# se-hwan/landing-controller

Hardware: AMD Instinct MI355X
Metric: landing NLPs solved/sec (SRBM, N=40, batch) (higher is better)
Workload: dtype f64

## Files before the change

landing-controller_amd/csrc/layout.hpp:

```cpp
#pragma once

namespace landing {

struct Layout {
  int N;
  int nx, ng, np, nnz_jac, nnz_hess;
  int o_dt, o_q_min, o_q_max, o_qd_min, o_qd_max, o_q_init, o_qd_init, o_q_term_min, o_q_term_max,
      o_qd_term_min, o_qd_term_max, o_QN, o_mu, o_l_leg_max, o_f_max, o_mass, o_Ib, o_Ib_inv;
  int o_Uref, o_QX, o_Qc, o_Qf;
  double kin_box[3], kin_z_off, comp_eps, slip_eps;
  int run_cost;
  double QX[12], Qc[3], Qf[3], f_ref[3], p_hip[12];

  __host__ __device__ int x_X(int k) const { return 12 * k; }
  __host__ __device__ int x_U(int k) const { return 12 * (N + 1) + 24 * k; }
  __host__ __device__ int g_stage(int k) const { return 36 + 104 * k; }
  __host__ __device__ int rows(int k) const { return k == N - 1 ? 80 : 104; }
  __host__ __device__ int jx(int k) const { return 157 * k; }
  __host__ __device__ int ju(int k) const { return 157 * N + 36 + (k == 0 ? 0 : 204 + 228 * (k - 1)); }
  __host__ __device__ int ju_len(int k) const { return k == 0 ? (N == 1 ? 156 : 204) : (k == N - 1 ? 180 : 228); }
  __host__ __device__ int hx(int k) const { return 29 * k; }
  __host__ __device__ int hu(int k) const { return 29 * N + 12 + (k == 0 ? 0 : 148 + 160 * (k - 1)); }
};

inline Layout make_layout(int N) {
  Layout L;
  L.N = N;
  L.nx = 36 * N + 12; L.ng = 104 * N + 12; L.np = 13 * N + 94;
  L.nnz_jac = 36 + 385 * (N - 1) + 313; L.nnz_hess = 177 * N + 12 * (N - 1) + 12;
  L.o_dt = 12 * (N + 1);
  const int b = L.o_dt + N;
  L.o_q_min = b; L.o_q_max = b + 6; L.o_qd_min = b + 12; L.o_qd_max = b + 18; L.o_q_init = b + 24; L.o_qd_init = b + 30;
  L.o_q_term_min = b + 36; L.o_q_term_max = b + 42; L.o_qd_term_min = b + 48; L.o_qd_term_max = b + 54;
  L.o_QN = b + 60; L.o_mu = b + 72; L.o_l_leg_max = b + 73; L.o_f_max = b + 74; L.o_mass = b + 75; L.o_Ib = b + 76; L.o_Ib_inv = b + 79;
  L.kin_box[0] = 0.15; L.kin_box[1] = 0.15; L.kin_box[2] = 0.30; L.kin_z_off = 0.05; L.comp_eps = 1e-3; L.slip_eps = 1e-2;
  L.run_cost = 0;
  L.o_Uref = L.o_QX = L.o_Qc = L.o_Qf = -1;
  { const double ph[12] = {0.19, -0.1, -0.2, 0.19, 0.1, -0.2, -0.19, -0.1, -0.2, -0.19, 0.1, -0.2};
    for (int i = 0; i < 12; ++i) { L.QX[i] = 0.0; L.p_hip[i] = ph[i]; }
    for (int i = 0; i < 3; ++i) { L.Qc[i] = 0.0; L.Qf[i] = 0.0; L.f_ref[i] = 0.0; } }
  return L;
}

inline void layout_ccc_params(Layout& L) {
  const int N = L.N;
  L.run_cost = 2;
  L.o_Uref = 12 * (N + 1);
  L.o_dt = L.o_Uref + 24 * N;
  const int b = L.o_dt + N;
  L.o_q_min = b; L.o_q_max = b + 6; L.o_qd_min = b + 12; L.o_qd_max = b + 18; L.o_q_init = b + 24; L.o_qd_init = b + 30;
  L.o_q_term_min = b + 36; L.o_q_term_max = b + 42; L.o_qd_term_min = b + 48; L.o_qd_term_max = b + 54;
  L.o_QX = b + 60; L.o_QN = b + 72; L.o_Qc = b + 84; L.o_Qf = b + 87;
  L.o_mu = b + 90; L.o_l_leg_max = b + 91; L.o_f_max = b + 92; L.o_mass = b + 93; L.o_Ib = b + 94; L.o_Ib_inv = b + 97;
  L.np = b + 100;
}

}
```

landing-controller_amd/csrc/solver_kernels.hip:

```cpp
#include <hip/hip_runtime.h>
#include <math.h>
#include <type_traits>

#include "../../include/landing_nlp.h"
#include "ipm_core.hpp"


namespace landing {

constexpr int NZ_JX = 0, NZ_JU = 157, NZ_JUN = 385, NZ_HX = 613, NZ_HU = 642, NZ_HUN = 802, NZ_TOT = 962;
constexpr int GS = 49;
constexpr int PS = 25;
constexpr int YS = 37;
constexpr int RIC_K = 0, RIC_KAP = 576, RIC_MT = 600, RIC_MV = 888, RIC_PX = 900, RIC_PV = 1188, RIC_STRIDE = 1200;
constexpr int RIC_FWD0 = 288, RIC_FWDN = 612;
constexpr int FILT_CAP = 64;
constexpr int SOLVER_NMAX = 96;
constexpr int SOLVER_THREADS = 256;
constexpr int RCG = 36;
constexpr int RUNC = 48;

constexpr int CX_SR = NZ_TOT + 48, CX_ONE = CX_SR + 208, CX_MONE = CX_ONE + 1, CX_ZERO = CX_ONE + 2, CX_LEN = CX_ONE + 3;
constexpr int ATAB_TB = 6, ATAB_LTMAX = 6;
constexpr int ASM_NSLOT = 512;
// ... 107 lines not shown
#pragma unroll
  for (int i = 0; i < MEMBER_MEM_PTRS; ++i) {
    const unsigned long long a = (unsigned long long)q[i];
    const unsigned lo = (unsigned)__builtin_amdgcn_readfirstlane((int)(unsigned)a), hi = (unsigned)__builtin_amdgcn_readfirstlane((int)(unsigned)(a >> 32));
    q[i] = (double*)((unsigned long long)lo | ((unsigned long long)hi << 32));
  }
#endif
  return M;
}
static_assert(36 * FWD_DXL_NMAX + 12 <= 24 * PS + 2 * XCH + 2 * 12 * YS && offsetof(Lds, A1) == offsetof(Lds, P) + sizeof(double) * 24 * PS && offsetof(Lds, Ah) == offsetof(Lds, A1) + sizeof(double) * 2 * XCH,
              "dx (x layout, N <= FWD_DXL_NMAX) fits the adjacent arrays [P | A1 | A^] (forward_pass / row_products)");
static_assert(offsetof(Lds, atab_mid) <= 65528, "the assembly tables address G, A^, gamma, cx, the partial sums and the dump slots with 16-bit byte offsets");
__host__ __device__ inline unsigned long long aterm_pack(int pa, int pb, int pc, int d, bool keep, bool ah) {
  const unsigned lo = (unsigned)pa | ((unsigned)pb << 16);
  const unsigned hi = (unsigned)pc | (((unsigned)d | (keep ? 1u : 0u) | (ah ? 2u : 0u)) << 16);
  return (unsigned long long)lo | ((unsigned long long)hi << 32);
}
__host__ __device__ inline unsigned long long acomb_pack(int n, int s0, int d, bool ah) {
  return (unsigned long long)((unsigned)n | ((unsigned)s0 << 16)) | ((unsigned long long)((unsigned)d | (ah ? 2u : 0u)) << 32);
}

template <int KT, class FA, class FB>
__device__ __forceinline__ f64x4 mfma_tile(f64x4 c, FA fa, FB fb) {
  const int l = threadIdx.x & 63, ij = l & 15, kq = l >> 4;
#pragma unroll
  for (int kt = 0; kt < KT; ++kt) c = __builtin_amdgcn_mfma_f64_16x16x4f64(fa(ij, kt * 4 + kq), fb(kt * 4 + kq, ij), c, 0, 0, 0);
  return c;
}

__device__ __forceinline__ double fast_rcp(double d) {
  double i = __builtin_amdgcn_rcp(d);
  i = fma(i, fma(-d, i, 1.0), i);
  return fma(i, fma(-d, i, 1.0), i);
}

__device__ __forceinline__ double lane_bcast(double v, int src) {
  const int hi = __builtin_amdgcn_readlane(__double2hiint(v), src);
  const int lo = __builtin_amdgcn_readlane(__double2loint(v), src);
  return __hiloint2double(hi, lo);
}

template <int NU>
__device__ __noinline__ void gauss_jordan_wave(const double* G, const double* gam, double* Kl, double* kl, int* flag) {
  const int lane = threadIdx.x;
  double col[NU];
  const bool isUU = lane < NU, isUS = lane >= NU && lane < NU + 24, isG = lane == NU + 24;
  {
    const double* src = isG ? gam + 24 : G + 24 * GS + (isUU ? 24 + lane : (isUS ? lane - NU : 0));
    const int stride = isG ? 1 : GS;
#pragma unroll
    for (int i = 0; i < NU; ++i) col[i] = src[i * stride];
  }
  bool ok = true;
#pragma unroll 1
  for (int j = 0; j < NU; ++j) {
    const double d = lane_bcast(col[0], j);
    if (!(d > 0.0) || !(d < 1e300)) ok = false;
    double inv = __builtin_amdgcn_rcp(d);
    inv = fma(inv, fma(-d, inv, 1.0), inv);
    inv = fma(inv, fma(-d, inv, 1.0), inv);
    const double pj = col[0] * inv;
    double m[NU];
#pragma unroll
    for (int i = 1; i < NU; ++i) m[i] = lane_bcast(col[i], j);
    __builtin_amdgcn_sched_barrier(0);
#pragma unroll
    for (int i = 1; i < NU; ++i) col[i - 1] = fma(-m[i], pj, col[i]);
    col[NU - 1] = pj;
  }
  if (isUS) {
#pragma unroll
    for (int i = 0; i < NU; ++i) Kl[i * 24 + (lane - NU)] = col[i];
  }
  if (isG) {
#pragma unroll
    for (int i = 0; i < NU; ++i) kl[i] = col[i];
  }
  if (lane == 0) *flag = ok ? 1 : 0;
}

constexpr int ASM_SEG_LEN[7] = {NZ_JU - NZ_JX, NZ_JUN - NZ_JU, NZ_HX - NZ_JUN, NZ_HU - NZ_HX, NZ_HUN - NZ_HU, NZ_TOT - NZ_HUN, RUNC};
constexpr int ASM_SEG_POS[7] = {NZ_JX, NZ_JU, NZ_JUN, NZ_HX, NZ_HU, NZ_HUN, NZ_TOT};
static_assert(NZ_JUN - NZ_JU <= SOLVER_THREADS && 2 * 104 <= SOLVER_THREADS, "one load per thread and segment");
struct AsmRegs { double jh[7], sr, g, rc; };
__device__ __forceinline__ void asm_issue(int k, AsmRegs& R) {
  const Lds& S = SH;
  const MemberMem& M = S.M;
  const int tid = threadIdx.x, ng = S.L.ng;
  landing_gptr JH = (landing_gptr)M.J;
  landing_gptr SR = (landing_gptr)M.sig;
  const int* sb = S.segb + k * 8;
  const int g0 = S.L.g_stage(k);
#pragma unroll
  for (int sgm = 0; sgm < 7; ++sgm) R.jh[sgm] = JH[sb[sgm] + (tid < ASM_SEG_LEN[sgm] ? tid : 0)];
  R.sr = SR[tid < 104 ? g0 + tid : (tid < 208 ? ng + g0 + tid - 104 : 0)];
  R.g = ((landing_gptr)M.g)[g0 + (tid < 12 ? tid : 0)];
  R.rc = 0.0;
  if (S.rc_on) R.rc = ((landing_gptr)M.cond)[(size_t)k * RCG + (tid < RCG ? tid : 0)];
}
__device__ __forceinline__ void asm_copy(const AsmRegs& R) {
  Lds& S = SH;
  const int tid = threadIdx.x;
#pragma unroll
  for (int sgm = 0; sgm < 7; ++sgm) if (tid < ASM_SEG_LEN[sgm]) S.jhl[ASM_SEG_POS[sgm] + tid] = R.jh[sgm];
  if (tid < 208) S.jhl[CX_SR + tid] = R.sr;
}
__device__ __forceinline__ void asm_terms(int k, int nb, const AsmRegs& R) {
  Lds& S = SH;
  const int tid = threadIdx.x, LT = S.c_ml, tp = S.segb[k * 8 + 7];
  char* const lds0 = reinterpret_cast<char*>(&S);
  const unsigned ahoff = nb ? (unsigned)(12 * YS * sizeof(double)) : 0u;
  const bool mid = (tp == S.c_mid);
  const unsigned long long* gt = S.ctab + (size_t)tp * LT * SOLVER_THREADS;
  double acc = 0.0;
  for (int j0 = 0; j0 < LT; j0 += ATAB_TB) {
    unsigned long long t[ATAB_TB];
    if (mid) {
#pragma unroll
      for (int u = 0; u < ATAB_TB; ++u) t[u] = S.atab_mid[(j0 + u) * SOLVER_THREADS + tid];
    } else {
#pragma unroll
      for (int u = 0; u < ATAB_TB; ++u) t[u] = gt[(j0 + u) * SOLVER_THREADS + tid];
    }
    double a[ATAB_TB], b[ATAB_TB], c[ATAB_TB];
#pragma unroll
    for (int u = 0; u < ATAB_TB; ++u) {
      const unsigned lo = (unsigned)t[u], hi = (unsigned)(t[u] >> 32);
      a[u] = *reinterpret_cast<const double*>(lds0 + (lo & 0xffffu)); b[u] = *reinterpret_cast<const double*>(lds0 + (lo >> 16)); c[u] = *reinterpret_cast<const double*>(lds0 + (hi & 0xffffu));
    }
#pragma unroll
    for (int u = 0; u < ATAB_TB; ++u) {
      const unsigned dd = (unsigned)(t[u] >> 48);
      acc += a[u] * b[u] * c[u];
      *reinterpret_cast<double*>(lds0 + ((dd & 0xfff8u) + ((dd & 2u) ? ahoff : 0u))) = acc;
      acc = (dd & 1u) ? acc : 0.0;
    }
  }
  if (tid < 12) { const int i = tid; S.Ah[nb * (12 * YS) + (i < 6 ? i : (i < 9 ? i + 3 : i - 3)) * YS + (YS - 1)] = -R.g; }
  if (tid < RCG) S.rcl[tid] = R.rc;
}
__device__ __forceinline__ void asm_combine(int k, int nb) {
  Lds& S = SH;
  const int tid = threadIdx.x, tp = S.segb[k * 8 + 7];
  const unsigned long long code = tp == S.c_mid ? S.acomb_mid[tid] : S.ccomb[tp * SOLVER_THREADS + tid];
  const unsigned lo = (unsigned)code, dd = (unsigned)(code >> 32);
  const int n = (int)(lo & 7u);
  if (n > 0) {
    char* const lds0 = reinterpret_cast<char*>(&S);
    const double* sl = reinterpret_cast<const double*>(lds0 + (lo >> 16));
    double tot = 0.0;
    for (int i = 0; i < n; ++i) tot += sl[i];
    *reinterpret_cast<double*>(lds0 + ((dd & 0xfff8u) + ((dd & 2u) ? (nb ? (unsigned)(12 * YS * sizeof(double)) : 0u) : 0u))) = tot;
  }
}

#if defined(__HIP_DEVICE_COMPILE__)
typedef double __attribute__((address_space(1)))* landing_gptr_w;
#else
typedef double* landing_gptr_w;
#endif
__device__ __forceinline__ landing_gptr_w uniform_record(double* rec) {
#if defined(__HIP_DEVICE_COMPILE__)
  const unsigned long long a = (unsigned long long)rec;
  const unsigned lo = (unsigned)__builtin_amdgcn_readfirstlane((int)(unsigned)a), hi = (unsigned)__builtin_amdgcn_readfirstlane((int)(unsigned)(a >> 32));
  return (landing_gptr_w)((unsigned long long)lo | ((unsigned long long)hi << 32));
#else
  return rec;
#endif
}

template <int STEP>
__device__ __forceinline__ bool pivot_block_step(f64x4 (&T)[3], int ct, int lj, int lk, int c) {
  constexpr int OFF = 4 * STEP;
  static_assert((OFF >> 4) == ((OFF + 3) >> 4), "a pivot block lies inside one row tile");
  Lds& S = SH;
  constexpr int RTB = OFF >> 4, R0 = (OFF & 15) >> 2;
  constexpr int WSZ = 64 * 4;
  static_assert(WSZ + 48 * 4 <= XCH, "exchange buffer");
  double* W = S.A1 + (STEP & 1) * XCH;
  double* C = W + WSZ;
#pragma unroll
  for (int q = 0; q < 1; ++q) W[c * 4 + 4 * q + lk] = T[RTB][R0 + q];
  if (ct == RTB && lj >= (OFF & 15) && lj < (OFF & 15) + 4) {
#pragma unroll
    for (int rt = 0; rt < 3; ++rt)
#pragma unroll
      for (int r = 0; r < 4; ++r) C[(16 * rt + lk + 4 * r) * 4 + (lj - (OFF & 15))] = T[rt][r];
  }
  __syncthreads();
  double a[4][4];
#pragma unroll
  for (int i = 0; i < 4; ++i)
#pragma unroll
    for (int j = 0; j <= i; ++j) a[i][j] = C[(OFF + i) * 4 + j];
  double w[4];
#pragma unroll
  for (int i = 0; i < 4; ++i) w[i] = W[c * 4 + i];
  double am[3];
#pragma unroll
  for (int rt = 0; rt < 3; ++rt) { const int row = 16 * rt + lj; const double cv = C[row * 4 + lk]; am[rt] = (row >= OFF && row < OFF + 4) ? 0.0 : cv; }
  auto recip = [](double d) { double i = __builtin_amdgcn_rcp(d); i = fma(i, fma(-d, i, 1.0), i); return fma(i, fma(-d, i, 1.0), i); };
  const double a00 = a[0][0], a10 = a[1][0], a11 = a[1][1], a20 = a[2][0], a21 = a[2][1], a22 = a[2][2], a30 = a[3][0], a31 = a[3][1], a32 = a[3][2], a33 = a[3][3];
  const double detA = fma(a00, a11, -a10 * a10), iA = recip(detA);
  const double e00 = fma(a20, a11, -a21 * a10) * iA, e01 = fma(a21, a00, -a20 * a10) * iA, e10 = fma(a30, a11, -a31 * a10) * iA, e11 = fma(a31, a00, -a30 * a10) * iA;
  const double s00 = fma(-e01, a21, fma(-e00, a20, a22)), s10 = fma(-e11, a21, fma(-e10, a20, a32)), s11 = fma(-e11, a31, fma(-e10, a30, a33));
  const double detS = fma(s00, s11, -s10 * s10), iS = recip(detS);
  unsigned hm = 0u;
  { const double piv[4] = {a00, detA, s00, detS};
#pragma unroll
    for (int j = 0; j < 4; ++j) { const unsigned h = (unsigned)__double2hiint(piv[j]) - 0x00100000u; hm = h > hm ? h : hm; } }
  const bool ok = hm < (0x7e37e43cu - 0x00100000u);
  auto solve = [&](const double (&wv)[4]) {
    const double t2 = fma(-e01, wv[1], fma(-e00, wv[0], wv[2])), t3 = fma(-e11, wv[1], fma(-e10, wv[0], wv[3]));
    const double r2 = fma(s11, t2, -s10 * t3) * iS, r3 = fma(s00, t3, -s10 * t2) * iS;
    const double q0 = fma(a11, wv[0], -a10 * wv[1]) * iA, q1 = fma(a00, wv[1], -a10 * wv[0]) * iA;
    const double r0 = fma(-e10, r3, fma(-e00, r2, q0)), r1 = fma(-e11, r3, fma(-e01, r2, q1));
    return lk == 0 ? r0 : (lk == 1 ? r1 : (lk == 2 ? r2 : r3));
  };
  const double R = solve(w);
  if (16 * ct + 16 > OFF) {
#pragma unroll
    for (int rt = 0; rt < 3; ++rt) T[rt] = __builtin_amdgcn_mfma_f64_16x16x4f64(am[rt], -R, T[rt], 0, 0, 0);
    T[RTB][R0] = R;
  }
  return ok;
}

constexpr int G_GAMMA = GS - 1, P_PV = PS - 1, AH_B = YS - 1;
static_assert(G_GAMMA == 48 && P_PV == 24 && AH_B == 36, "spare columns of G / P / A^ hold gamma / p / b");
template <int NU>
__device__ __noinline__ bool block_eliminate(double* __restrict__ rec_, double delta, int k) {
  Lds& S = SH;
  constexpr int NR = NU + 24;
  const int tid = threadIdx.x, ct = tid >> 6, l = tid & 63, lj = l & 15, lk = l >> 4;
  const int c = 16 * ct + lj;
  const bool isg = (c == NR), live = (c <= NR);
  const int cb = k & 1;
  f64x4 T[3];
  const double* const lds0 = reinterpret_cast<const double*>(&S);
  constexpr int oG = (int)(offsetof(Lds, G) / sizeof(double)), oP = (int)(offsetof(Lds, P) / sizeof(double));
  const int oAh = (int)(offsetof(Lds, Ah) / sizeof(double)) + cb * (12 * YS);
  const int cl = c < NR ? c : NR;
  const int cp = NU == 24 ? cl : (cl < NU ? cl : cl + (24 - NU));
  const bool ym = live && (c < 12 || c >= NU);
  int ycol = c < NU ? c + 24 : c - NU;
  ycol = ym ? (isg ? AH_B : ycol) : 0;
  const bool pm = live && c >= 12 && (c < NU || isg);
  const int pcol = pm ? (isg ? P_PV : c) : 0;
  {
    const int gb = oG + cp + lk * GS, cd = cp - lk, cm = c - lk;
#pragma unroll
    for (int rt = 0; rt < 3; ++rt)
#pragma unroll
      for (int r = 0; r < 4; ++r) {
        const int rb = 16 * rt + 4 * r;
        if (rb < NR) {
          const int rp = NU == 24 ? rb : (rb < NU ? rb : rb + (24 - NU));
          const int m = rp < cd ? rp : cd;
          const double v = lds0[gb + rp + (GS - 1) * m] + (cm == rb ? delta : 0.0);
          T[rt][r] = live ? v : 0.0;
        } else T[rt][r] = 0.0;
      }
    if (S.rc_on) {
#pragma unroll
      for (int rt = 0; rt < 3; ++rt)
#pragma unroll
        for (int r = 0; r < 4; ++r) {
          const int rb = 16 * rt + 4 * r;
          if (rb < NR) {
            const int ab = rb < NU ? 24 + rb : rb - NU;
            static_assert(RCG % 4 == 0 && NU % 4 == 0, "a group of four rows lies on one side of every border");
            const double g = ab < RCG ? S.rcl[ab + lk] : 0.0;
            T[rt][r] += isg ? g : 0.0;
          }
        }
    }
  }
  {
    double be[3];
    {
      const int yb = oAh + lk * YS + ycol;
#pragma unroll
      for (int kt = 0; kt < 3; ++kt) { const double v = lds0[yb + 4 * kt * YS]; be[kt] = ym ? v : 0.0; }
    }
    double pa1[3], add1[3];
#pragma unroll
    for (int kt = 0; kt < 3; ++kt) pa1[kt] = lds0[oP + lj * PS + 4 * kt + lk];
    const int pb = oP + lk * PS + pcol;
#pragma unroll
    for (int r = 0; r < 3; ++r) { const double v = lds0[pb + 4 * r * PS]; add1[r] = pm ? v : 0.0; }
    double av[3][3];
#pragma unroll
    for (int rt = 0; rt < 3; ++rt) {
      const int rho = 16 * rt + lj;
      const int a = rho < NU ? 24 + rho : (rho < NR ? rho - NU : 36);
      const bool am = a < 36;
      const int ab = oAh + lk * YS + (am ? a : 0);
#pragma unroll
      for (int kt = 0; kt < 3; ++kt) { const double v = lds0[ab + 4 * kt * YS]; av[rt][kt] = am ? v : 0.0; }
    }
    double pa2[3], add2[3];
    if (NU == 24) {
      const int p2 = oP + (12 + (lj < 12 ? lj : 11)) * PS + lk;
#pragma unroll
      for (int kt = 0; kt < 3; ++kt) pa2[kt] = lds0[p2 + 4 * kt];
#pragma unroll
      for (int r = 0; r < 3; ++r) { const double v = lds0[pb + (12 + 4 * r) * PS]; add2[r] = pm ? v : 0.0; }
    }
    f64x4 Y1 = {0.0, 0.0, 0.0, 0.0};
#pragma unroll
    for (int kt = 0; kt < 3; ++kt) Y1 = __builtin_amdgcn_mfma_f64_16x16x4f64(pa1[kt], be[kt], Y1, 0, 0, 0);
#pragma unroll
    for (int r = 0; r < 3; ++r) Y1[r] += add1[r];
#pragma unroll
    for (int rt = 0; rt < 3; ++rt)
#pragma unroll
      for (int kt = 0; kt < 3; ++kt) T[rt] = __builtin_amdgcn_mfma_f64_16x16x4f64(av[rt][kt], Y1[kt], T[rt], 0, 0, 0);
    if (NU == 24) {
      f64x4 Y2 = {0.0, 0.0, 0.0, 0.0};
#pragma unroll
      for (int kt = 0; kt < 3; ++kt) Y2 = __builtin_amdgcn_mfma_f64_16x16x4f64(pa2[kt], be[kt], Y2, 0, 0, 0);
#pragma unroll
      for (int r = 0; r < 3; ++r) Y2[r] += add2[r];
      T[0][3] += Y2[0]; T[1][0] += Y2[1]; T[1][1] += Y2[2];
    }
  }
  static_assert(NU == 12 || NU == 24, "3 or 6 block steps per stage");
  constexpr int SC = NU == 24 ? 3 : 1;
  AsmRegs nxt;
  const bool more = k > 0;
#define ASM_HOOK(step) do { if constexpr (SC == (step)) { if (more) asm_copy(nxt); } if constexpr (SC + 1 == (step)) { if (more) asm_terms(k - 1, cb ^ 1, nxt); } if constexpr (SC + 2 == (step)) { if (more) asm_combine(k - 1, cb ^ 1); } } while (0)
  bool ok = pivot_block_step<0>(T, ct, lj, lk, c);
  if (more) asm_issue(k - 1, nxt);
  ASM_HOOK(1);
  ok &= pivot_block_step<1>(T, ct, lj, lk, c);
  ASM_HOOK(2);
  ok &= pivot_block_step<2>(T, ct, lj, lk, c);
  ASM_HOOK(3);
  if constexpr (NU == 24) {
    ok &= pivot_block_step<3>(T, ct, lj, lk, c);
    ASM_HOOK(4);
    ok &= pivot_block_step<4>(T, ct, lj, lk, c);
    ASM_HOOK(5);
    ok &= pivot_block_step<5>(T, ct, lj, lk, c);
  }
#undef ASM_HOOK
  if (!ok) return false;
  f64x4 Mq = {0.0, 0.0, 0.0, 0.0};
  {
    const int fb = oAh + (lj < 12 ? lj : 11) * YS + 24 + lk;
#pragma unroll
    for (int kt = 0; kt < 3; ++kt) Mq = __builtin_amdgcn_mfma_f64_16x16x4f64(lds0[fb + 4 * kt], T[0][kt], Mq, 0, 0, 0);
  }
  if (c >= NU && c <= NR) {
    const unsigned sj = (unsigned)(c - NU), ulk = (unsigned)lk;
    const unsigned rs = isg ? 1u : 24u;
    const unsigned iK = (isg ? (unsigned)RIC_KAP : (unsigned)RIC_K + sj) + ulk * rs, iM = (isg ? (unsigned)RIC_MV : (unsigned)RIC_MT + sj) + ulk * rs,
                   iP = (isg ? (unsigned)RIC_PV : (unsigned)RIC_PX + sj) + ulk * rs;
    const int scol = isg ? AH_B : (int)sj, pcw = isg ? P_PV : (int)sj;
    landing_gptr_w rec = uniform_record(rec_);
    double* const Pw = S.P + lk * PS + pcw;
#pragma unroll
    for (int r = 0; r < 3; ++r) rec[iM + (unsigned)(4 * r) * rs] = lds0[oAh + (lk + 4 * r) * YS + scol] - Mq[r];
#pragma unroll
    for (int rt = 0; rt < 3; ++rt)
#pragma unroll
      for (int r = 0; r < 4; ++r) {
        const int rb = 16 * rt + 4 * r;
        const double v = T[rt][r];
        if (rb < NU) rec[iK + (unsigned)rb * rs] = v;
        else if (rb < NR) {
          Pw[(rb - NU) * PS] = v;
          if (rb - NU < 12) rec[iP + (unsigned)(rb - NU) * rs] = v;
        }
      }
  }
  return true;
}

template <int NU>
__device__ __forceinline__ bool riccati_step(double* rec, double delta, int k) {
  const bool ok = block_eliminate<NU>(rec, delta, k);
  __syncthreads();
  return ok;
}

__device__ __noinline__ bool riccati_backward(double delta) {
  Lds& S = SH;
  const Layout& L = S.L;
  const MemberMem& M = S.M;
  const double* p = S.p;
  const int N = L.N, lane = threadIdx.x, NT = blockDim.x;
  (void)p; (void)N; (void)lane; (void)NT;
  bool ok = true;
  int n_try = 0;
  for (int e = lane; e < 24 * PS; e += NT) S.P[e] = 0.0;
  __syncthreads();
  if (lane < 12) {
    const int i = lane;
    const int ra = i < 6 ? 12 + i : 24 + (i - 6), rb = i < 6 ? 18 + i : 30 + (i - 6);
    const double qn2 = S.ks.feas ? 0.0 : 2.0 * p[L.o_QN + i];
    S.P[i * PS + i] = qn2 + M.sig[ra] + M.sig[rb] + delta;
    S.P[i * PS + P_PV] = qn2 * (M.x[12 * N + i] - p[12 * N + i]) + M.rho[ra] + M.rho[rb];
    double* rec = M.ric + (size_t)N * RIC_STRIDE;
    for (int j = 0; j < 24; ++j) rec[RIC_PX + i * 24 + j] = (j == i) ? S.P[i * PS + i] : 0.0;
    rec[RIC_PV + i] = S.P[i * PS + P_PV];
  }
  for (int e = lane; e < 48 * GS; e += NT) S.G[e] = 0.0;
  for (int e = lane; e < 2 * 12 * YS; e += NT) S.Ah[e] = 0.0;
  __syncthreads();
  {
    AsmRegs first;
    asm_issue(N - 1, first);
    asm_copy(first);
    __syncthreads();
    asm_terms(N - 1, (N - 1) & 1, first);
    __syncthreads();
    asm_combine(N - 1, (N - 1) & 1);
  }
  __syncthreads();
  for (int k = N - 1; k >= 0 && ok; --k) {
    const bool last = (k == N - 1);
    long long tb_ = S.prof_on ? (long long)wall_clock64() : 0;
    double* rec = M.ric + (size_t)k * RIC_STRIDE;
    ok = last ? riccati_step<12>(rec, delta, k) : riccati_step<24>(rec, delta, k);
    ++n_try;
    PROF_ADD(PH_B_ELIM, tb_);
  }
  if (ok) {
    if (lane < 12) {
      const int i = lane;
      const double x0i = (i < 6) ? p[L.o_q_init + i] : p[L.o_qd_init + i - 6];
      S.sig[i] = x0i - M.x[i];
    }
    for (int e = lane; e < 144; e += NT) { const int i = e / 12, j = e % 12; S.G[(24 + i) * GS + 24 + j] = S.P[(12 + i) * PS + 12 + j]; }
    __syncthreads();
    if (lane < 12) {
      double v = S.P[(12 + lane) * PS + P_PV];
      for (int t = 0; t < 12; ++t) v += S.P[(12 + lane) * PS + t] * S.sig[t];
      S.gam[24 + lane] = v;
    }
    __syncthreads();
    if (lane < 64) gauss_jordan_wave<12>(S.G, S.gam, S.A1, S.A1 + 24 * 24, &S.flag);
    __syncthreads();
    ok = S.flag != 0;
    ++n_try;
    if (ok) {
      if (lane < 12) S.sig[12 + lane] = -S.A1[24 * 24 + lane];
      __syncthreads();
    }
  }
  if (lane == 0) { S.prof[PH_NSTAGE] += (double)n_try; S.prof[PH_NSTAGE_OK] += (double)(ok ? n_try : n_try - 1); }
  __syncthreads();
  return ok;
}

__device__ __noinline__ void forward_pass() {
  Lds& S = SH;
  const Layout& L = S.L;
  const MemberMem& M = S.M;
  const int N = L.N, tid = threadIdx.x, NT = blockDim.x;
  double* sg = S.G;
  double* buf = S.jhl;
  double* buf1 = S.A1;
  static_assert(24 * (SOLVER_NMAX + 1) <= 48 * GS && RIC_FWDN <= NZ_TOT + RUNC && RIC_FWDN <= XCH * 2, "forward scratch fits");
  auto slot = [&](int k) { return (k & 1) ? buf1 : buf; };
  auto fetch = [&](int k, double (&r)[3]) {
    landing_gptr rec = (landing_gptr)(M.ric + (size_t)(k < N ? k : N - 1) * RIC_STRIDE + RIC_FWD0);
#pragma unroll
    for (int j = 0; j < 3; ++j) { const int e = tid + j * 256; r[j] = rec[e < RIC_FWDN ? e : RIC_FWDN - 1]; }
  };
  auto stash = [&](int k, const double (&r)[3]) {
    double* b = slot(k);
#pragma unroll
    for (int j = 0; j < 3; ++j) { const int e = tid + j * 256; if (k < N && e < RIC_FWDN) b[e] = r[j]; }
  };
  if (tid < 24) sg[tid] = S.sig[tid];
  double r0[3], r1[3], r2[3], r3[3];
  fetch(0, r0); fetch(1, r1); fetch(2, r2); fetch(3, r3);
  stash(0, r0); fetch(4, r0);
  __syncthreads();
  auto stage = [&](int k, double (&rn)[3]) {
    if (k < N) {
      const double* b = slot(k);
      const bool lastk = (k == N - 1);
      if (tid < 192) {
        const int r = tid >> 3, j = tid & 7;
        const double* row = (r < 12) ? b + 312 + r * 24 : b + (r - 12) * 24;
        const double* sk = sg + 24 * k;
        double acc = row[3 * j] * sk[3 * j] + row[3 * j + 1] * sk[3 * j + 1] + row[3 * j + 2] * sk[3 * j + 2];
        acc += __shfl_xor(acc, 1); acc += __shfl_xor(acc, 2); acc += __shfl_xor(acc, 4);
        if (j == 0) sg[24 * (k + 1) + r] = (r < 12) ? b[600 + r] + acc : (lastk ? 0.0 : -(b[300 + (r - 12)] + acc));
      }
    }
    stash(k + 1, rn);
    fetch(k + 5, rn);
    __syncthreads();
  };
  for (int k0 = 0; k0 < N; k0 += 4) {
    stage(k0, r1); stage(k0 + 1, r2); stage(k0 + 2, r3); stage(k0 + 3, r0);
  }
  double* const dxl = S.P;
  const bool use_dxl = N <= FWD_DXL_NMAX;
  for (int e = tid; e < 24 * (N + 1); e += NT) {
    const int k = e / 24, i = e % 24;
    if (i < 12) { M.dx[L.x_X(k) + i] = sg[e]; if (use_dxl) dxl[L.x_X(k) + i] = sg[e]; }
    else if (k < N) { M.dx[L.x_U(k) + (i - 12)] = sg[e]; if (use_dxl) dxl[L.x_U(k) + (i - 12)] = sg[e]; }
  }
  for (int e = tid; e < 24 * N; e += NT) {
    const int k = e / 24, h = e % 24, i = h % 12;
// ... 730 lines not shown
```

Measured before the change: 21900.

## Hoist per-stage lane addressing and uniform context out of Riccati backward loop

Adds a stage-invariant lane descriptor (byte offsets into LDS and record addresses) that is computed once, plus a readfirstlane-uniformized context of global pointers and scalars, so the per-stage elimination loop no longer recomputes indices or reloads shared metadata. The noinline block_eliminate call per stage becomes an inlined loop with the last stage split out. Pivot checks now reduce a max key rather than ANDing booleans. The aim is to cut scalar/vector ALU overhead and call cost in the serial backward sweep, at the cost of extra register pressure from the hoisted descriptor.

Result: faster. 22510 (median of 6 runs) (+2.8%).

```diff
diff --git a/landing-controller_amd/csrc/layout.hpp b/landing-controller_amd/csrc/layout.hpp
--- a/landing-controller_amd/csrc/layout.hpp
+++ b/landing-controller_amd/csrc/layout.hpp
@@ -14,7 +14,7 @@
 
   __host__ __device__ int x_X(int k) const { return 12 * k; }
   __host__ __device__ int x_U(int k) const { return 12 * (N + 1) + 24 * k; }
-  __host__ __device__ int g_stage(int k) const { return 36 + 104 * k; }
+  __host__ __device__ static constexpr int g_stage(int k) { return 36 + 104 * k; }
   __host__ __device__ int rows(int k) const { return k == N - 1 ? 80 : 104; }
   __host__ __device__ int jx(int k) const { return 157 * k; }
   __host__ __device__ int ju(int k) const { return 157 * N + 36 + (k == 0 ? 0 : 204 + 228 * (k - 1)); }
diff --git a/landing-controller_amd/csrc/solver_kernels.hip b/landing-controller_amd/csrc/solver_kernels.hip
--- a/landing-controller_amd/csrc/solver_kernels.hip
+++ b/landing-controller_amd/csrc/solver_kernels.hip
@@ -213,21 +213,45 @@
 constexpr int ASM_SEG_LEN[7] = {NZ_JU - NZ_JX, NZ_JUN - NZ_JU, NZ_HX - NZ_JUN, NZ_HU - NZ_HX, NZ_HUN - NZ_HU, NZ_TOT - NZ_HUN, RUNC};
 constexpr int ASM_SEG_POS[7] = {NZ_JX, NZ_JU, NZ_JUN, NZ_HX, NZ_HU, NZ_HUN, NZ_TOT};
 static_assert(NZ_JUN - NZ_JU <= SOLVER_THREADS && 2 * 104 <= SOLVER_THREADS, "one load per thread and segment");
-struct AsmRegs { double jh[7], sr, g, rc; };
-__device__ __forceinline__ void asm_issue(int k, AsmRegs& R) {
+__device__ __forceinline__ int uni(int v) {
+#if defined(__HIP_DEVICE_COMPILE__)
+  return __builtin_amdgcn_readfirstlane(v);
+#else
+  return v;
+#endif
+}
+template <class P>
+__device__ __forceinline__ P uni_ptr(P q) {
+  const unsigned long long a = (unsigned long long)q;
+  return (P)((unsigned long long)(unsigned)uni((int)(unsigned)a) | ((unsigned long long)(unsigned)uni((int)(unsigned)(a >> 32)) << 32));
+}
+__device__ __forceinline__ double uni(double v) { return __hiloint2double(uni(__double2hiint(v)), uni(__double2loint(v))); }
+struct SweepCtx {
+  landing_gptr JH, SR, Gr, Cd;
+  const unsigned long long* ctab; const unsigned long long* ccomb;
+  int c_ml, c_mid, rc_on, ng;
+};
+__device__ __forceinline__ SweepCtx sweep_ctx() {
   const Lds& S = SH;
-  const MemberMem& M = S.M;
-  const int tid = threadIdx.x, ng = S.L.ng;
-  landing_gptr JH = (landing_gptr)M.J;
-  landing_gptr SR = (landing_gptr)M.sig;
+  SweepCtx X;
+  X.JH = uni_ptr((landing_gptr)S.M.J); X.SR = uni_ptr((landing_gptr)S.M.sig); X.Gr = uni_ptr((landing_gptr)S.M.g); X.Cd = uni_ptr((landing_gptr)S.M.cond);
+  X.ctab = uni_ptr(S.ctab); X.ccomb = uni_ptr(S.ccomb);
+  X.c_ml = uni(S.c_ml); X.c_mid = uni(S.c_mid); X.rc_on = uni(S.rc_on); X.ng = uni(S.L.ng);
+  return X;
+}
+struct AsmRegs { double jh[7], sr, g, rc; int tp; };
+__device__ __forceinline__ void asm_issue(int k, const SweepCtx& X, AsmRegs& R) {
+  const Lds& S = SH;
+  const int tid = threadIdx.x, ng = X.ng;
   const int* sb = S.segb + k * 8;
-  const int g0 = S.L.g_stage(k);
-#pragma unroll
-  for (int sgm = 0; sgm < 7; ++sgm) R.jh[sgm] = JH[sb[sgm] + (tid < ASM_SEG_LEN[sgm] ? tid : 0)];
-  R.sr = SR[tid < 104 ? g0 + tid : (tid < 208 ? ng + g0 + tid - 104 : 0)];
-  R.g = ((landing_gptr)M.g)[g0 + (tid < 12 ? tid : 0)];
+  const int g0 = Layout::g_stage(k);
+#pragma unroll
+  for (int sgm = 0; sgm < 7; ++sgm) R.jh[sgm] = X.JH[uni(sb[sgm]) + (tid < ASM_SEG_LEN[sgm] ? tid : 0)];
+  R.tp = uni(sb[7]);
+  R.sr = X.SR[tid < 104 ? g0 + tid : (tid < 208 ? ng + g0 + tid - 104 : 0)];
+  R.g = X.Gr[g0 + (tid < 12 ? tid : 0)];
   R.rc = 0.0;
-  if (S.rc_on) R.rc = ((landing_gptr)M.cond)[(size_t)k * RCG + (tid < RCG ? tid : 0)];
+  if (X.rc_on) R.rc = X.Cd[(size_t)k * RCG + (tid < RCG ? tid : 0)];
 }
 __device__ __forceinline__ void asm_copy(const AsmRegs& R) {
   Lds& S = SH;
@@ -236,13 +260,13 @@
   for (int sgm = 0; sgm < 7; ++sgm) if (tid < ASM_SEG_LEN[sgm]) S.jhl[ASM_SEG_POS[sgm] + tid] = R.jh[sgm];
   if (tid < 208) S.jhl[CX_SR + tid] = R.sr;
 }
-__device__ __forceinline__ void asm_terms(int k, int nb, const AsmRegs& R) {
+__device__ __forceinline__ void asm_terms(const SweepCtx& X, int nb, const AsmRegs& R) {
   Lds& S = SH;
-  const int tid = threadIdx.x, LT = S.c_ml, tp = S.segb[k * 8 + 7];
+  const int tid = threadIdx.x, LT = X.c_ml, tp = R.tp;
   char* const lds0 = reinterpret_cast<char*>(&S);
   const unsigned ahoff = nb ? (unsigned)(12 * YS * sizeof(double)) : 0u;
-  const bool mid = (tp == S.c_mid);
-  const unsigned long long* gt = S.ctab + (size_t)tp * LT * SOLVER_THREADS;
+  const bool mid = (tp == X.c_mid);
+  const unsigned long long* gt = X.ctab + (size_t)tp * LT * SOLVER_THREADS;
   double acc = 0.0;
   for (int j0 = 0; j0 < LT; j0 += ATAB_TB) {
     unsigned long long t[ATAB_TB];
@@ -270,10 +294,10 @@
   if (tid < 12) { const int i = tid; S.Ah[nb * (12 * YS) + (i < 6 ? i : (i < 9 ? i + 3 : i - 3)) * YS + (YS - 1)] = -R.g; }
   if (tid < RCG) S.rcl[tid] = R.rc;
 }
-__device__ __forceinline__ void asm_combine(int k, int nb) {
+__device__ __forceinline__ void asm_combine(const SweepCtx& X, int nb, const AsmRegs& R) {
   Lds& S = SH;
-  const int tid = threadIdx.x, tp = S.segb[k * 8 + 7];
-  const unsigned long long code = tp == S.c_mid ? S.acomb_mid[tid] : S.ccomb[tp * SOLVER_THREADS + tid];
+  const int tid = threadIdx.x, tp = R.tp;
+  const unsigned long long code = tp == X.c_mid ? S.acomb_mid[tid] : X.ccomb[tp * SOLVER_THREADS + tid];
   const unsigned lo = (unsigned)code, dd = (unsigned)(code >> 32);
   const int n = (int)(lo & 7u);
   if (n > 0) {
@@ -290,46 +314,96 @@
 #else
 typedef double* landing_gptr_w;
 #endif
-__device__ __forceinline__ landing_gptr_w uniform_record(double* rec) {
-#if defined(__HIP_DEVICE_COMPILE__)
-  const unsigned long long a = (unsigned long long)rec;
-  const unsigned lo = (unsigned)__builtin_amdgcn_readfirstlane((int)(unsigned)a), hi = (unsigned)__builtin_amdgcn_readfirstlane((int)(unsigned)(a >> 32));
-  return (landing_gptr_w)((unsigned long long)lo | ((unsigned long long)hi << 32));
-#else
-  return rec;
-#endif
-}
-
-template <int STEP>
-__device__ __forceinline__ bool pivot_block_step(f64x4 (&T)[3], int ct, int lj, int lk, int c) {
-  constexpr int OFF = 4 * STEP;
+__device__ __forceinline__ landing_gptr_w uniform_record(double* rec) { return uni_ptr((landing_gptr_w)rec); }
+
+constexpr int G_GAMMA = GS - 1, P_PV = PS - 1, AH_B = YS - 1;
+static_assert(G_GAMMA == 48 && P_PV == 24 && AH_B == 36, "spare columns of G / P / A^ hold gamma / p / b");
+
+template <int NU>
+struct StageLanes {
+  int ct, lj, lk, c;
+  bool isg, live, ym, pm, wr;
+  bool am[3];
+  int gb, cd384, cm;
+  int yb, pa1, pb, p2, fb, ab[3];
+  int xw, xw0, xcp, xcr;
+  unsigned iK, iM, iP, rs;
+  int sw, pw;
+};
+template <int NU>
+__device__ __forceinline__ StageLanes<NU> stage_lanes() {
+  constexpr int NR = NU + 24, D = (int)sizeof(double);
+  constexpr int oG = (int)offsetof(Lds, G), oP = (int)offsetof(Lds, P), oAh = (int)offsetof(Lds, Ah), oA1 = (int)offsetof(Lds, A1);
+  StageLanes<NU> Z;
+  const int tid = threadIdx.x, l = tid & 63;
+  Z.ct = uni(tid >> 6); Z.lj = l & 15; Z.lk = l >> 4;
+  const int ct = Z.ct, lj = Z.lj, lk = Z.lk, c = 16 * ct + lj;
+  Z.c = c;
+  Z.isg = (c == NR); Z.live = (c <= NR);
+  const bool isg = Z.isg, live = Z.live;
+  const int cl = c < NR ? c : NR;
+  const int cp = NU == 24 ? cl : (cl < NU ? cl : cl + (24 - NU));
+  Z.ym = live && (c < 12 || c >= NU);
+  int ycol = c < NU ? c + 24 : c - NU;
+  ycol = Z.ym ? (isg ? AH_B : ycol) : 0;
+  Z.pm = live && c >= 12 && (c < NU || isg);
+  const int pcol = Z.pm ? (isg ? P_PV : c) : 0;
+  Z.gb = oG + (cp + lk * GS) * D; Z.cd384 = (cp - lk) * ((GS - 1) * D); Z.cm = c - lk;
+  Z.yb = oAh + (lk * YS + ycol) * D;
+  Z.pa1 = oP + (lj * PS + lk) * D;
+  Z.pb = oP + (lk * PS + pcol) * D;
+#pragma unroll
+  for (int rt = 0; rt < 3; ++rt) {
+    const int rho = 16 * rt + lj;
+    const int a = rho < NU ? 24 + rho : (rho < NR ? rho - NU : 36);
+    Z.am[rt] = a < 36;
+    Z.ab[rt] = oAh + (lk * YS + (Z.am[rt] ? a : 0)) * D;
+  }
+  Z.p2 = oP + ((12 + (lj < 12 ? lj : 11)) * PS + lk) * D;
+  Z.fb = oAh + ((lj < 12 ? lj : 11) * YS + 24 + lk) * D;
+  Z.xw = oA1 + (c * 4 + lk) * D; Z.xw0 = oA1 + (c * 4) * D; Z.xcp = oA1 + (64 * 4 + lk * 4 + lj) * D; Z.xcr = oA1 + (64 * 4 + lj * 4 + lk) * D;
+  Z.wr = c >= NU && c <= NR;
+  const unsigned sj = (unsigned)(c - NU), ulk = (unsigned)lk, rs = isg ? 1u : 24u;
+  Z.rs = rs * D;
+  Z.iK = ((isg ? (unsigned)RIC_KAP : (unsigned)RIC_K + sj) + ulk * rs) * D; Z.iM = ((isg ? (unsigned)RIC_MV : (unsigned)RIC_MT + sj) + ulk * rs) * D;
+  Z.iP = ((isg ? (unsigned)RIC_PV : (unsigned)RIC_PX + sj) + ulk * rs) * D;
+  const int scol = isg ? AH_B : (int)sj, pcw = isg ? P_PV : (int)sj;
+  Z.sw = oAh + (lk * YS + scol) * D; Z.pw = oP + (lk * PS + pcw) * D;
+  return Z;
+}
+__device__ __forceinline__ double lds_get(int boff) { return *reinterpret_cast<const double*>(reinterpret_cast<const char*>(&SH) + boff); }
+__device__ __forceinline__ void lds_put(int boff, double v) { *reinterpret_cast<double*>(reinterpret_cast<char*>(&SH) + boff) = v; }
+
+constexpr unsigned PIVOT_KEY_MAX = 0x7e37e43cu - 0x00100000u;
+template <int STEP, int NU>
+__device__ __forceinline__ unsigned pivot_block_step(f64x4 (&T)[3], const StageLanes<NU>& Z) {
+  constexpr int OFF = 4 * STEP, D = (int)sizeof(double);
   static_assert((OFF >> 4) == ((OFF + 3) >> 4), "a pivot block lies inside one row tile");
-  Lds& S = SH;
   constexpr int RTB = OFF >> 4, R0 = (OFF & 15) >> 2;
   constexpr int WSZ = 64 * 4;
   static_assert(WSZ + 48 * 4 <= XCH, "exchange buffer");
-  double* W = S.A1 + (STEP & 1) * XCH;
-  double* C = W + WSZ;
-#pragma unroll
-  for (int q = 0; q < 1; ++q) W[c * 4 + 4 * q + lk] = T[RTB][R0 + q];
-  if (ct == RTB && lj >= (OFF & 15) && lj < (OFF & 15) + 4) {
+  constexpr int XB = (STEP & 1) * XCH * D;
+  constexpr int CB = (int)offsetof(Lds, A1) + XB + WSZ * D;
+  const bool inblk = (unsigned)(Z.lj - (OFF & 15)) < 4u;
+  lds_put(Z.xw + XB, T[RTB][R0]);
+  if (Z.ct == RTB && inblk) {
 #pragma unroll
     for (int rt = 0; rt < 3; ++rt)
 #pragma unroll
-      for (int r = 0; r < 4; ++r) C[(16 * rt + lk + 4 * r) * 4 + (lj - (OFF & 15))] = T[rt][r];
+      for (int r = 0; r < 4; ++r) lds_put(Z.xcp + XB + ((16 * rt + 4 * r) * 4 - (OFF & 15)) * D, T[rt][r]);
   }
   __syncthreads();
   double a[4][4];
 #pragma unroll
   for (int i = 0; i < 4; ++i)
 #pragma unroll
-    for (int j = 0; j <= i; ++j) a[i][j] = C[(OFF + i) * 4 + j];
+    for (int j = 0; j <= i; ++j) a[i][j] = lds_get(CB + ((OFF + i) * 4 + j) * D);
   double w[4];
 #pragma unroll
-  for (int i = 0; i < 4; ++i) w[i] = W[c * 4 + i];
+  for (int i = 0; i < 4; ++i) w[i] = lds_get(Z.xw0 + XB + i * D);
   double am[3];
 #pragma unroll
-  for (int rt = 0; rt < 3; ++rt) { const int row = 16 * rt + lj; const double cv = C[row * 4 + lk]; am[rt] = (row >= OFF && row < OFF + 4) ? 0.0 : cv; }
+  for (int rt = 0; rt < 3; ++rt) { const double cv = lds_get(Z.xcr + XB + 16 * rt * 4 * D); am[rt] = (rt == RTB && inblk) ? 0.0 : cv; }
   auto recip = [](double d) { double i = __builtin_amdgcn_rcp(d); i = fma(i, fma(-d, i, 1.0), i); return fma(i, fma(-d, i, 1.0), i); };
   const double a00 = a[0][0], a10 = a[1][0], a11 = a[1][1], a20 = a[2][0], a21 = a[2][1], a22 = a[2][2], a30 = a[3][0], a31 = a[3][1], a32 = a[3][2], a33 = a[3][3];
   const double detA = fma(a00, a11, -a10 * a10), iA = recip(detA);
@@ -340,7 +414,7 @@
   { const double piv[4] = {a00, detA, s00, detS};
 #pragma unroll
     for (int j = 0; j < 4; ++j) { const unsigned h = (unsigned)__double2hiint(piv[j]) - 0x00100000u; hm = h > hm ? h : hm; } }
-  const bool ok = hm < (0x7e37e43cu - 0x00100000u);
+  const int lk = Z.lk;
   auto solve = [&](const double (&wv)[4]) {
     const double t2 = fma(-e01, wv[1], fma(-e00, wv[0], wv[2])), t3 = fma(-e11, wv[1], fma(-e10, wv[0], wv[3]));
     const double r2 = fma(s11, t2, -s10 * t3) * iS, r3 = fma(s00, t3, -s10 * t2) * iS;
@@ -349,37 +423,31 @@
     return lk == 0 ? r0 : (lk == 1 ? r1 : (lk == 2 ? r2 : r3));
   };
   const double R = solve(w);
-  if (16 * ct + 16 > OFF) {
+  if (16 * Z.ct + 16 > OFF) {
 #pragma unroll
     for (int rt = 0; rt < 3; ++rt) T[rt] = __builtin_amdgcn_mfma_f64_16x16x4f64(am[rt], -R, T[rt], 0, 0, 0);
     T[RTB][R0] = R;
   }
-  return ok;
-}
-
-constexpr int G_GAMMA = GS - 1, P_PV = PS - 1, AH_B = YS - 1;
-static_assert(G_GAMMA == 48 && P_PV == 24 && AH_B == 36, "spare columns of G / P / A^ hold gamma / p / b");
+  return hm;
+}
+
+__device__ __forceinline__ void rec_put(landing_gptr_w rec, unsigned boff, double v) {
+#if defined(__HIP_DEVICE_COMPILE__)
+  typedef char __attribute__((address_space(1)))* gchar_w;
+  *reinterpret_cast<landing_gptr_w>(reinterpret_cast<gchar_w>(rec) + boff) = v;
+#else
+  *reinterpret_cast<double*>(reinterpret_cast<char*>(rec) + boff) = v;
+#endif
+}
 template <int NU>
-__device__ __noinline__ bool block_eliminate(double* __restrict__ rec_, double delta, int k) {
-  Lds& S = SH;
-  constexpr int NR = NU + 24;
-  const int tid = threadIdx.x, ct = tid >> 6, l = tid & 63, lj = l & 15, lk = l >> 4;
-  const int c = 16 * ct + lj;
-  const bool isg = (c == NR), live = (c <= NR);
+__device__ __forceinline__ bool stage_eliminate(const StageLanes<NU>& Z, const SweepCtx& X, landing_gptr_w rec, double delta, int k) {
+  constexpr int NR = NU + 24, D = (int)sizeof(double);
+  const int lk = Z.lk;
+  const bool isg = Z.isg, live = Z.live, ym = Z.ym, pm = Z.pm;
   const int cb = k & 1;
+  const int ah = cb * (12 * YS * D);
   f64x4 T[3];
-  const double* const lds0 = reinterpret_cast<const double*>(&S);
-  constexpr int oG = (int)(offsetof(Lds, G) / sizeof(double)), oP = (int)(offsetof(Lds, P) / sizeof(double));
-  const int oAh = (int)(offsetof(Lds, Ah) / sizeof(double)) + cb * (12 * YS);
-  const int cl = c < NR ? c : NR;
-  const int cp = NU == 24 ? cl : (cl < NU ? cl : cl + (24 - NU));
-  const bool ym = live && (c < 12 || c >= NU);
-  int ycol = c < NU ? c + 24 : c - NU;
-  ycol = ym ? (isg ? AH_B : ycol) : 0;
-  const bool pm = live && c >= 12 && (c < NU || isg);
-  const int pcol = pm ? (isg ? P_PV : c) : 0;
   {
-    const int gb = oG + cp + lk * GS, cd = cp - lk, cm = c - lk;
 #pragma unroll
     for (int rt = 0; rt < 3; ++rt)
 #pragma unroll
@@ -387,12 +455,13 @@
         const int rb = 16 * rt + 4 * r;
         if (rb < NR) {
           const int rp = NU == 24 ? rb : (rb < NU ? rb : rb + (24 - NU));
-          const int m = rp < cd ? rp : cd;
-          const double v = lds0[gb + rp + (GS - 1) * m] + (cm == rb ? delta : 0.0);
+          const int m384 = rp * ((GS - 1) * D) < Z.cd384 ? rp * ((GS - 1) * D) : Z.cd384;
+          const double v = lds_get(Z.gb + rp * D + m384) + (Z.cm == rb ? delta : 0.0);
           T[rt][r] = live ? v : 0.0;
         } else T[rt][r] = 0.0;
       }
-    if (S.rc_on) {
+    if (X.rc_on) {
+      Lds& S = SH;
 #pragma unroll
       for (int rt = 0; rt < 3; ++rt)
 #pragma unroll
@@ -410,33 +479,28 @@
   {
     double be[3];
     {
-      const int yb = oAh + lk * YS + ycol;
-#pragma unroll
-      for (int kt = 0; kt < 3; ++kt) { const double v = lds0[yb + 4 * kt * YS]; be[kt] = ym ? v : 0.0; }
+      const int yb = Z.yb + ah;
+#pragma unroll
+      for (int kt = 0; kt < 3; ++kt) { const double v = lds_get(yb + 4 * kt * YS * D); be[kt] = ym ? v : 0.0; }
     }
     double pa1[3], add1[3];
 #pragma unroll
-    for (int kt = 0; kt < 3; ++kt) pa1[kt] = lds0[oP + lj * PS + 4 * kt + lk];
-    const int pb = oP + lk * PS + pcol;
-#pragma unroll
-    for (int r = 0; r < 3; ++r) { const double v = lds0[pb + 4 * r * PS]; add1[r] = pm ? v : 0.0; }
+    for (int kt = 0; kt < 3; ++kt) pa1[kt] = lds_get(Z.pa1 + 4 * kt * D);
+#pragma unroll
+    for (int r = 0; r < 3; ++r) { const double v = lds_get(Z.pb + 4 * r * PS * D); add1[r] = pm ? v : 0.0; }
     double av[3][3];
 #pragma unroll
     for (int rt = 0; rt < 3; ++rt) {
-      const int rho = 16 * rt + lj;
-      const int a = rho < NU ? 24 + rho : (rho < NR ? rho - NU : 36);
-      const bool am = a < 36;
-      const int ab = oAh + lk * YS + (am ? a : 0);
-#pragma unroll
-      for (int kt = 0; kt < 3; ++kt) { const double v = lds0[ab + 4 * kt * YS]; av[rt][kt] = am ? v : 0.0; }
+      const int ab = Z.ab[rt] + ah;
+#pragma unroll
+      for (int kt = 0; kt < 3; ++kt) { const double v = lds_get(ab + 4 * kt * YS * D); av[rt][kt] = Z.am[rt] ? v : 0.0; }
     }
     double pa2[3], add2[3];
     if (NU == 24) {
-      const int p2 = oP + (12 + (lj < 12 ? lj : 11)) * PS + lk;
-#pragma unroll
-      for (int kt = 0; kt < 3; ++kt) pa2[kt] = lds0[p2 + 4 * kt];
-#pragma unroll
-      for (int r = 0; r < 3; ++r) { const double v = lds0[pb + (12 + 4 * r) * PS]; add2[r] = pm ? v : 0.0; }
+#pragma unroll
+      for (int kt = 0; kt < 3; ++kt) pa2[kt] = lds_get(Z.p2 + 4 * kt * D);
+#pragma unroll
+      for (int r = 0; r < 3; ++r) { const double v = lds_get(Z.pb + (12 + 4 * r) * PS * D); add2[r] = pm ? v : 0.0; }
     }
     f64x4 Y1 = {0.0, 0.0, 0.0, 0.0};
 #pragma unroll
@@ -460,59 +524,68 @@
   constexpr int SC = NU == 24 ? 3 : 1;
   AsmRegs nxt;
   const bool more = k > 0;
-#define ASM_HOOK(step) do { if constexpr (SC == (step)) { if (more) asm_copy(nxt); } if constexpr (SC + 1 == (step)) { if (more) asm_terms(k - 1, cb ^ 1, nxt); } if constexpr (SC + 2 == (step)) { if (more) asm_combine(k - 1, cb ^ 1); } } while (0)
-  bool ok = pivot_block_step<0>(T, ct, lj, lk, c);
-  if (more) asm_issue(k - 1, nxt);
+#define ASM_HOOK(step) do { if constexpr (SC == (step)) { if (more) asm_copy(nxt); } if constexpr (SC + 1 == (step)) { if (more) asm_terms(X, cb ^ 1, nxt); } if constexpr (SC + 2 == (step)) { if (more) asm_combine(X, cb ^ 1, nxt); } } while (0)
+  unsigned key = pivot_block_step<0>(T, Z), kq;
+#define KEY_MAX(e) do { kq = (e); key = kq > key ? kq : key; } while (0)
+  if (more) asm_issue(k - 1, X, nxt);
   ASM_HOOK(1);
-  ok &= pivot_block_step<1>(T, ct, lj, lk, c);
+  KEY_MAX(pivot_block_step<1>(T, Z));
   ASM_HOOK(2);
-  ok &= pivot_block_step<2>(T, ct, lj, lk, c);
+  KEY_MAX(pivot_block_step<2>(T, Z));
   ASM_HOOK(3);
   if constexpr (NU == 24) {
-    ok &= pivot_block_step<3>(T, ct, lj, lk, c);
+    KEY_MAX(pivot_block_step<3>(T, Z));
     ASM_HOOK(4);
-    ok &= pivot_block_step<4>(T, ct, lj, lk, c);
+    KEY_MAX(pivot_block_step<4>(T, Z));
     ASM_HOOK(5);
-    ok &= pivot_block_step<5>(T, ct, lj, lk, c);
-  }
+    KEY_MAX(pivot_block_step<5>(T, Z));
+  }
+#undef KEY_MAX
 #undef ASM_HOOK
-  if (!ok) return false;
+  if (!((unsigned)uni((int)key) < PIVOT_KEY_MAX)) return false;
   f64x4 Mq = {0.0, 0.0, 0.0, 0.0};
   {
-    const int fb = oAh + (lj < 12 ? lj : 11) * YS + 24 + lk;
-#pragma unroll
-    for (int kt = 0; kt < 3; ++kt) Mq = __builtin_amdgcn_mfma_f64_16x16x4f64(lds0[fb + 4 * kt], T[0][kt], Mq, 0, 0, 0);
-  }
-  if (c >= NU && c <= NR) {
-    const unsigned sj = (unsigned)(c - NU), ulk = (unsigned)lk;
-    const unsigned rs = isg ? 1u : 24u;
-    const unsigned iK = (isg ? (unsigned)RIC_KAP : (unsigned)RIC_K + sj) + ulk * rs, iM = (isg ? (unsigned)RIC_MV : (unsigned)RIC_MT + sj) + ulk * rs,
-                   iP = (isg ? (unsigned)RIC_PV : (unsigned)RIC_PX + sj) + ulk * rs;
-    const int scol = isg ? AH_B : (int)sj, pcw = isg ? P_PV : (int)sj;
-    landing_gptr_w rec = uniform_record(rec_);
-    double* const Pw = S.P + lk * PS + pcw;
-#pragma unroll
-    for (int r = 0; r < 3; ++r) rec[iM + (unsigned)(4 * r) * rs] = lds0[oAh + (lk + 4 * r) * YS + scol] - Mq[r];
+    const int fb = Z.fb + ah;
+#pragma unroll
+    for (int kt = 0; kt < 3; ++kt) Mq = __builtin_amdgcn_mfma_f64_16x16x4f64(lds_get(fb + 4 * kt * D), T[0][kt], Mq, 0, 0, 0);
+  }
+  if (Z.wr) {
+    const int sw = Z.sw + ah;
+#pragma unroll
+    for (int r = 0; r < 3; ++r) rec_put(rec, Z.iM + (unsigned)(4 * r) * Z.rs, lds_get(sw + 4 * r * YS * D) - Mq[r]);
 #pragma unroll
     for (int rt = 0; rt < 3; ++rt)
 #pragma unroll
       for (int r = 0; r < 4; ++r) {
         const int rb = 16 * rt + 4 * r;
         const double v = T[rt][r];
-        if (rb < NU) rec[iK + (unsigned)rb * rs] = v;
+        if (rb < NU) rec_put(rec, Z.iK + (unsigned)rb * Z.rs, v);
         else if (rb < NR) {
-          Pw[(rb - NU) * PS] = v;
-          if (rb - NU < 12) rec[iP + (unsigned)(rb - NU) * rs] = v;
+          lds_put(Z.pw + (rb - NU) * PS * D, v);
+          if (rb - NU < 12) rec_put(rec, Z.iP + (unsigned)(rb - NU) * Z.rs, v);
         }
       }
   }
   return true;
 }
 
-template <int NU>
-__device__ __forceinline__ bool riccati_step(double* rec, double delta, int k) {
-  const bool ok = block_eliminate<NU>(rec, delta, k);
-  __syncthreads();
+__device__ __noinline__ bool last_stage_eliminate(double* rec_, double delta_, int k_) {
+  const StageLanes<12> Z = stage_lanes<12>();
+  const SweepCtx X = sweep_ctx();
+  return stage_eliminate<12>(Z, X, uniform_record(rec_), uni(delta_), uni(k_));
+}
+
+template <bool TIMED>
+__device__ __forceinline__ bool stage_loop(const StageLanes<24>& Z, const SweepCtx& X, landing_gptr_w rec, double delta, int k, int& n_try) {
+  bool ok = true;
+  for (; k >= 0 && ok; --k, rec -= RIC_STRIDE) {
+    long long tb_ = 0;
+    if (TIMED) tb_ = (long long)wall_clock64();
+    ok = stage_eliminate<24>(Z, X, rec, delta, k);
+    __syncthreads();
+    ++n_try;
+    if (TIMED) { const long long n_ = (long long)wall_clock64(); if (threadIdx.x == 0) SH.prof[PH_B_ELIM] += (double)(n_ - tb_); }
+  }
   return ok;
 }
 
@@ -540,23 +613,31 @@
   for (int e = lane; e < 48 * GS; e += NT) S.G[e] = 0.0;
   for (int e = lane; e < 2 * 12 * YS; e += NT) S.Ah[e] = 0.0;
   __syncthreads();
+  const SweepCtx X = sweep_ctx();
+  const bool timed = uni(S.prof_on) != 0;
   {
     AsmRegs first;
-    asm_issue(N - 1, first);
+    asm_issue(N - 1, X, first);
     asm_copy(first);
     __syncthreads();
-    asm_terms(N - 1, (N - 1) & 1, first);
+    asm_terms(X, (N - 1) & 1, first);
     __syncthreads();
-    asm_combine(N - 1, (N - 1) & 1);
+    asm_combine(X, (N - 1) & 1, first);
   }
   __syncthreads();
-  for (int k = N - 1; k >= 0 && ok; --k) {
-    const bool last = (k == N - 1);
-    long long tb_ = S.prof_on ? (long long)wall_clock64() : 0;
-    double* rec = M.ric + (size_t)k * RIC_STRIDE;
-    ok = last ? riccati_step<12>(rec, delta, k) : riccati_step<24>(rec, delta, k);
+  {
+    long long tb_ = timed ? (long long)wall_clock64() : 0;
+    ok = uni(last_stage_eliminate(M.ric + (size_t)(N - 1) * RIC_STRIDE, delta, N - 1) ? 1 : 0) != 0;
+    __syncthreads();
     ++n_try;
-    PROF_ADD(PH_B_ELIM, tb_);
+    if (timed) { const long long n_ = (long long)wall_clock64(); if (lane == 0) S.prof[PH_B_ELIM] += (double)(n_ - tb_); }
+  }
+  if (ok && N > 1) {
+    const StageLanes<24> Z = stage_lanes<24>();
+    const int Nu = uni(N);
+    const landing_gptr_w rec = uniform_record(M.ric) + (size_t)(Nu - 2) * RIC_STRIDE;
+    const double du = uni(delta);
+    ok = timed ? stage_loop<true>(Z, X, rec, du, Nu - 2, n_try) : stage_loop<false>(Z, X, rec, du, Nu - 2, n_try);
   }
   if (ok) {
     if (lane < 12) {
```
